# dashpay/agora-blsful

Measured on AMD Instinct MI355X. Metric: BLS12-381 sig verifications/sec (batch), higher is better.
Workload: dtype u32

## Files before the change

agora-blsful_amd/csrc/blsgpu.hip:

```cpp
#include <hip/hip_runtime.h>
#include <stdio.h>
#include <stdlib.h>
#include <string.h>
#include <algorithm>
#include <atomic>
#include <chrono>
#include <mutex>
#include <numeric>
#include <string>
#include <thread>
#include <type_traits>
#include <unordered_map>
#include <vector>

#include "../../include/blsgpu.h"
#include "kernels.cuh"
#include "shares.cuh"
#include "secure.cuh"
#include "agg_batch.cuh"
#include "host_sha256.h"

namespace {

const uint32_t FP_ONE_HOST[12] = FP_RAW_ONE_WORDS;
thread_local std::string t_err;
thread_local size_t t_devidx = 0;
thread_local bool t_nested = false;

enum {
  KID_PREPARE, KID_MILLER2, KID_FINALEXP, KID_PREPARE_AGG, KID_PAIRS_AFF, KID_MILLER1, KID_F12_FOLD, KID_FINALEXP_ONE,
  KID_HASH, KID_ACCUM, KID_POINT_FOLD, KID_COMPRESS, KID_SIGN, KID_F12_IO, KID_MSM_SORT, KID_MSM_BUCKET, KID_MSM_CHUNK, KID_DECOMPRESS, KID_PAIRING_COOP, KID_KEY_SORT, KID_COEFF, KID_DUP, KID_FIRST_BAD, KID_MSM_PREP, KID_MSM_NORM, KID_MSM_MERGE, KID_WIDE, KID_LINES, KID_CYCRUN,
  KID_MILLER2_V1, KID_FINALEXP_V1, KID_LINESP, KID_LINESP4, KID_LINE_QUAD, KID_F12_FOLD4, KID_F12_TREE, KID_HORNER, KID_MILLERFP, KID_PAIRING_POST, KID_PAIRING_PRE,
  KID_TAIL,
  KID_SHARE_LAGRANGE, KID_SHARE_LADDER, KID_SHARE_FOLD, KID_SHARE_OUT,
  KID_SECURE_RANK, KID_SECURE_GATHER, KID_SECURE_DIGEST, KID_SECURE_COEFF, KID_SECURE_OUT, KID_SECURE_FIN,
  KID_AGG_SEG_INDEX, KID_AGG_SEG_FOLD, KID_AGG_SEG_FIN,
  KID_COUNT
};
const char* KID_NAMES[KID_COUNT] = {"k_prepare", "k_millerf2s", "k_finalexp2s", "k_prepare_agg", "k_pairs_to_affine", "k_miller1s", "k_f12_fold",
                                    "k_finalexp_one", "k_hash_to_point", "k_accumulate", "k_point_fold", "k_compress", "k_sign", "k_f12_io", "k_msm_sort", "k_msm_bucket", "k_msm_chunk", "k_decompress", "k_pairing_coop", "k_key_sort", "k_sha256_coeff", "k_duplicate_rule", "k_first_identity", "k_msm_prep", "k_normalize", "k_msm_merge", "k_wide", "k_lines2s", "k_cyc_run4",
                                    "k_miller2s", "k_finalexps", "k_linesp", "k_linesp4", "k_line_quad", "k_f12_fold4", "k_f12_tree_seg", "k_f12_horner_wide", "k_millerfp", "k_pairing_post", "k_pairing_pre",
                                    "tail_stream_overlapped", "k_share_lagrange", "k_share_ladder", "k_share_fold", "k_share_out",
                                    "k_secure_rank", "k_secure_gather", "k_secure_digest", "k_secure_coeff", "k_secure_out", "k_secure_fin",
                                    "k_agg_seg_index", "k_f12_fold_seg", "k_agg_batch_fin"};

struct Ctx {
  int dev = -1;
  hipStream_t stream = nullptr;
  uint8_t* arena = nullptr;
  size_t arena_cap = 0, arena_off = 0;
  std::mutex mu;
  hipEvent_t ev_host = nullptr;
  hipStream_t side = nullptr;
  hipEvent_t ev_fork = nullptr, ev_join = nullptr;
  hipStream_t side2 = nullptr;
  hipEvent_t ev_join2 = nullptr;
  uint8_t* hpin = nullptr;
  size_t hpin_cap = 0;
  uint8_t* hsmall = nullptr;
  size_t hsmall_off = 0;
  hipStream_t tail = nullptr;
  hipEvent_t ev_tail_fork = nullptr, ev_tail_join = nullptr;
  uint32_t* fold_ws = nullptr;
  uint32_t* lines_ws = nullptr;
  size_t lines_cap = 0;
  uint32_t* stream_flags = nullptr;
  uint32_t stream_epoch = 0;
  bool prof_on = false;
  struct Pending { int kid; hipEvent_t e0, e1; };
  std::vector<Pending> prof_pending;
  std::vector<hipEvent_t> prof_pool;
  double prof_ms[KID_COUNT] = {0};
  uint64_t prof_cnt[KID_COUNT] = {0};
};
struct Device {
  int dev = -1;
  std::vector<Ctx*> pool;
// ... 34 lines not shown
  Ctx* c = d->pool[d->rr.fetch_add(1) % d->pool.size()];
  L.lk = std::unique_lock<std::mutex>(c->mu);
  L.c = c;
  return L;
}
#define CTX_ACQUIRE_ON(c, devidx)        \
  Lease lease_ = acquire_ctx(devidx);     \
  Ctx* c = lease_.c;                      \
  c->hsmall_off = 0;                      \
  HIPCK(hipSetDevice(c->dev))
#define CTX_ACQUIRE(c) CTX_ACQUIRE_ON(c, t_devidx)
#define NOT_INIT() fail(BLSGPU_E_NOT_INIT, "blsgpu_init has not been called (or found no gfx950 device)")
#define API_CATCH                                                                              \
  catch (const std::bad_alloc&) { return fail(BLSGPU_E_HIP, "out of host memory"); }           \
  catch (const std::exception& e) { return fail(BLSGPU_E_HIP, std::string("internal: ") + e.what()); } \
  catch (...) { return fail(BLSGPU_E_HIP, "internal: unknown exception"); }

int fail(int code, const std::string& msg) {
  t_err = msg;
  return code;
}
extern "C" char** environ;
struct Knobs {
  long coop_max = 4096, wide_max = 512, shard_min = 8192, contexts = 2, fake_devices = 0, acc_lanes = 57344;
  long msm_c = 0, msm_ch = 0, msm2_c = 0, msm2_ch = 0, msm2_q = 0;
  long msm2_tables = 1;
  long stream_lines = 1;
  long post_split = 3;
  long host_trace = 0, strict_env = 0, ab_knobs = 0;
  long shares_msm_min = 1024;
  long secure_batch_max = 1024;
  long agg_batch_max = 32768;
  long ws_keep_mb = 4096;
  long miller_chunk = 65536, miller_v1 = 0, row_pad = 192, wide_mode = 2, finalexp_seg = 0, finalexp_v1 = 0, prepare_lanes = 0, product_tree = 1,
       tree_local = 0, lines4_max = -1, tree_engine_from = 0, agg_lanes = 0, msm_v1 = 0, msm_naive = 0, wide_test_block = 64;
  std::string problem;
};
struct KnobSpec { const char* name; long Knobs::*field; long lo, hi; bool ab; };
const KnobSpec KNOB_TABLE[] = {
    {"BLSGPU_COOP_MAX", &Knobs::coop_max, 0, 1 << 20, false},          {"BLSGPU_WIDE_MAX", &Knobs::wide_max, 0, 4096, false},
    {"BLSGPU_SHARD_MIN", &Knobs::shard_min, 1, 1L << 40, false},        {"BLSGPU_CONTEXTS", &Knobs::contexts, 1, 16, false},
    {"BLSGPU_FAKE_DEVICES", &Knobs::fake_devices, 0, 64, false},        {"BLSGPU_ACC_LANES", &Knobs::acc_lanes, 64, 1 << 20, false},
    {"BLSGPU_MSM_C", &Knobs::msm_c, 4, 16, false},                      {"BLSGPU_MSM_CH", &Knobs::msm_ch, 1, 1 << 16, false},
    {"BLSGPU_MSM2_C", &Knobs::msm2_c, 4, 16, false},                    {"BLSGPU_MSM2_CH", &Knobs::msm2_ch, 1, 1 << 16, false},
    {"BLSGPU_MSM2_Q", &Knobs::msm2_q, 1, 8, false},                     {"BLSGPU_HOST_TRACE", &Knobs::host_trace, 0, 1, false},
    {"BLSGPU_WS_KEEP_MB", &Knobs::ws_keep_mb, 0, 1L << 20, false},        {"BLSGPU_MSM2_TABLES", &Knobs::msm2_tables, 0, 1, false},
    {"BLSGPU_STREAM_LINES", &Knobs::stream_lines, 0, 1, false},        {"BLSGPU_POST_SPLIT", &Knobs::post_split, 0, 3, false},
    {"BLSGPU_STRICT_ENV", &Knobs::strict_env, 0, 1, false},             {"BLSGPU_AB_KNOBS", &Knobs::ab_knobs, 0, 1, false},
    {"BLSGPU_SHARES_MSM_MIN", &Knobs::shares_msm_min, 2, 1L << 32, false},
    {"BLSGPU_SECURE_BATCH_MAX", &Knobs::secure_batch_max, 1, 1L << 32, false},
    {"BLSGPU_AGG_BATCH_MAX", &Knobs::agg_batch_max, 1, 1L << 32, false},
    {"BLSGPU_MILLER_CHUNK", &Knobs::miller_chunk, 0, 65536, true},      {"BLSGPU_MILLER_V1", &Knobs::miller_v1, 0, 1, true},
    {"BLSGPU_ROW_PAD", &Knobs::row_pad, 0, 4096, true},                 {"BLSGPU_WIDE_MODE", &Knobs::wide_mode, 1, 2, true},
    {"BLSGPU_FINALEXP_SEG", &Knobs::finalexp_seg, 0, 1, true},          {"BLSGPU_FINALEXP_V1", &Knobs::finalexp_v1, 0, 1, true},
    {"BLSGPU_PREPARE_LANES", &Knobs::prepare_lanes, 0, 2, true},        {"BLSGPU_PRODUCT_TREE", &Knobs::product_tree, 0, 1, true},
    {"BLSGPU_TREE_LOCAL", &Knobs::tree_local, 0, 65536, true},          {"BLSGPU_LINES4_MAX", &Knobs::lines4_max, 0, 65536, true},
    {"BLSGPU_TREE_ENGINE_FROM", &Knobs::tree_engine_from, 0, 256, true}, {"BLSGPU_AGG_LANES", &Knobs::agg_lanes, 0, 2, true},
    {"BLSGPU_MSM_V1", &Knobs::msm_v1, 0, 1, true},                      {"BLSGPU_MSM_NAIVE", &Knobs::msm_naive, 0, 1, true},
    {"BLSGPU_WIDE_TEST_BLOCK", &Knobs::wide_test_block, 64, 256, true},
};
const char* const KNOB_OTHER_NAMES[] = {"BLSGPU_LIB", "BLSGPU_HASH_STOP"};
Knobs parse_knobs() {
  Knobs k;
  const char* gate = getenv("BLSGPU_AB_KNOBS");
  const bool ab_ok = gate && atol(gate) == 1;
  for (const KnobSpec& sp : KNOB_TABLE) {
    const char* e = getenv(sp.name);
    if (!e || !*e) continue;
    if (sp.ab && !ab_ok) {
      if (k.problem.empty()) k.problem = std::string(sp.name) + " is an A/B switch and needs BLSGPU_AB_KNOBS=1";
      fprintf(stderr, "libblsgpu: ignoring %s (an A/B switch: set BLSGPU_AB_KNOBS=1 to honour it)\n", sp.name);
      continue;
    }
    char* end = nullptr;
    long v = strtol(e, &end, 10);
    if (end == e || *end) {
      if (k.problem.empty()) k.problem = std::string(sp.name) + " is not an integer";
      continue;
    }
    k.*sp.field = v < sp.lo ? sp.lo : v > sp.hi ? sp.hi : v;
  }
  for (char** e = environ; e && *e; e++) {
    if (strncmp(*e, "BLSGPU_", 7) != 0) continue;
    const char* eq = strchr(*e, '=');
    const std::string name(*e, eq ? (size_t)(eq - *e) : strlen(*e));
    bool known = false;
    for (const KnobSpec& sp : KNOB_TABLE) known = known || name == sp.name;
    for (const char* o : KNOB_OTHER_NAMES) known = known || name == o;
    if (!known && k.problem.empty()) k.problem = "unknown variable " + name;
  }
  return k;
}
// ... 385 lines not shown
    c->lines_cap = 0;
  }
}

void launch_finalexp_chunk(Ctx* c, size_t n, size_t first, size_t cnt, const uint32_t* d_f, int32_t* d_status, bool seg) {
  const size_t nlanes = lanes_for(cnt), lanes = row_stride(nlanes);
  const dim3 grid((unsigned)(nlanes / BLS_BLOCK));
  if (seg) {
    const dim3 grid4(blocks_for(4 * cnt));
    for (int s = 0; s <= 5; s++) {
      KL(KID_FINALEXP, k_finalexp_seg, grid, dim3(BLS_BLOCK), s, n, first, cnt, d_f, c->lines_ws, lanes, d_status);
      if (s < 5) KL(KID_CYCRUN, k_cyc_run4, grid4, dim3(BLS_BLOCK), cnt, c->lines_ws, lanes, (const int32_t*)d_status, first);
    }
  } else {
    KL(KID_FINALEXP, k_finalexp2s, grid, dim3(BLS_BLOCK), n, first, cnt, d_f, c->lines_ws, lanes, d_status);
  }
}

int run_pairing2(Ctx* c, size_t n, uint32_t* d_pairs, uint32_t* d_f, int32_t* d_status, int fixed_g2) {
  if (n <= wide_max_items() && n <= coop_max_items()) {
    if (knobs().wide_mode == 1) {
      uint32_t* d_easy = (uint32_t*)arena_take(c, (size_t)WIDE_EASY_WORDS * 4 * n);
      if (!d_easy) return fail(BLSGPU_E_HIP, "internal: arena too small");
      KL(KID_PAIRING_COOP, k_pairing_coop_easy, dim3((unsigned)n), dim3(BLS_BLOCK), n, (const uint32_t*)d_pairs, (const int32_t*)d_status, fixed_g2, d_easy);
      KL(KID_WIDE, k_finalexp_wide, dim3((unsigned)n), dim3(WIDE_ENGINE_BLOCK), n, (const uint32_t*)d_easy, d_status);
    } else {
      KL(KID_WIDE, k_pairing_wide, dim3((unsigned)n), dim3(WIDE_ENGINE_BLOCK), n, (const uint32_t*)d_pairs, d_status, fixed_g2);
    }
  } else if (n <= coop_max_items()) {
    KL(KID_PAIRING_COOP, k_pairing_coop, dim3((unsigned)n), dim3(BLS_BLOCK), n, d_pairs, d_status, fixed_g2);
  } else {
    const bool finalexp_seg = knobs().finalexp_seg != 0;
    const bool finalexp_v1 = knobs().finalexp_v1 != 0;
    const size_t chunk = n < miller_chunk_items() ? n : miller_chunk_items();
    const size_t words_per_lane = (size_t)MILLER_ENTRIES * (LINE5_WORDS + (fixed_g2 ? 0 : LINE3_WORDS_H));
    if (chunk && lines_reserve(c, words_per_lane * 4 * row_stride(lanes_for(chunk))) == 0) {
      for (size_t first = 0; first < n; first += chunk) {
        const size_t cnt = n - first < chunk ? n - first : chunk;
        const size_t nlanes = lanes_for(cnt), lanes = row_stride(nlanes);
        uint32_t* lines3 = c->lines_ws + (size_t)MILLER_ENTRIES * LINE5_WORDS * lanes;
        const dim3 grid((unsigned)(nlanes / BLS_BLOCK));
        if (fixed_g2) {
          KL(KID_LINES, k_lines2s, grid, dim3(BLS_BLOCK), n, first, cnt, (const uint32_t*)d_pairs, (const int32_t*)d_status, c->lines_ws, lines3, lanes, fixed_g2, 0);
        } else {
          KL(KID_LINES, k_lines2s, grid, dim3(BLS_BLOCK), n, first, cnt, (const uint32_t*)d_pairs, (const int32_t*)d_status, c->lines_ws, lines3, lanes, 0, 1);
          KL(KID_LINES, k_lines2s, grid, dim3(BLS_BLOCK), n, first, cnt, (const uint32_t*)d_pairs, (const int32_t*)d_status, c->lines_ws, lines3, lanes, 0, 2);
        }
        KL(KID_MILLER2, k_millerf2s, grid, dim3(BLS_BLOCK), n, first, cnt, (const int32_t*)d_status, (const uint32_t*)c->lines_ws, lanes, d_f);
        if (!finalexp_v1) launch_finalexp_chunk(c, n, first, cnt, d_f, d_status, finalexp_seg);
      }
      if (finalexp_v1) KL(KID_FINALEXP_V1, k_finalexps, dim3(blocks_for(2 * n)), dim3(BLS_BLOCK), n, d_f, d_status);
    } else {
      KL(KID_MILLER2_V1, k_miller2s, dim3(blocks_for(2 * n)), dim3(BLS_BLOCK), n, d_pairs, d_status, d_f, fixed_g2);
      KL(KID_FINALEXP_V1, k_finalexps, dim3(blocks_for(2 * n)), dim3(BLS_BLOCK), n, d_f, d_status);
    }
  }
  HIPCK(hipGetLastError());
  return 0;
}

int side_fork(Ctx* c, int which = 3) {
  if (!c->side) {
    HIPCK(hipStreamCreateWithFlags(&c->side, hipStreamNonBlocking));
    HIPCK(hipEventCreateWithFlags(&c->ev_fork, hipEventDisableTiming));
    HIPCK(hipEventCreateWithFlags(&c->ev_join, hipEventDisableTiming));
    HIPCK(hipStreamCreateWithFlags(&c->side2, hipStreamNonBlocking));
    HIPCK(hipEventCreateWithFlags(&c->ev_join2, hipEventDisableTiming));
  }
  if (which & 1) HIPCK(hipEventRecord(c->ev_fork, c->stream));
  if (which & 2) {
    HIPCK(hipStreamWaitEvent(c->side, c->ev_fork, 0));
    HIPCK(hipStreamWaitEvent(c->side2, c->ev_fork, 0));
  }
  return 0;
}

void launch_hash_g1_small(hipStream_t stream, size_t n, const uint8_t* d_msgs, const uint64_t* d_offs, int flags, const dst_arg& dst, uint8_t* d_out,
                          uint32_t* d_rec) {
  if (n <= 128 && hash_phase_stop() == 0)
// ... 981 lines not shown
      cnt += c->prof_cnt[kernel_id];
    }
  if (total_ms) *total_ms = ms;
  if (launches) *launches = cnt;
  return 0;
}
API_CATCH

size_t blsgpu_last_error(char* buf, size_t cap) {
  if (buf && cap) {
    size_t k = std::min(cap - 1, t_err.size());
    memcpy(buf, t_err.data(), k);
    buf[k] = 0;
  }
  return t_err.size();
}

int blsgpu_verify_batch(int sig_group, int scheme, const void* pks, const void* sigs, const uint8_t* msgs,
                        const uint64_t* msg_offsets, size_t n, int fmt, int32_t* status) try {
  const bool wire = fmt == BLSGPU_FMT_COMPRESSED || fmt == BLSGPU_FMT_LEGACY;
  int rc = check_common(sig_group, scheme, wire ? BLSGPU_FMT_RAW_PROJ : fmt);
  if (rc) return rc;
  if (n == 0) return 0;
  if (!pks || !sigs || !msg_offsets || !status) return fail(BLSGPU_E_ARG, "null argument");
  if (const size_t D = shard_devices(n, {pks, sigs, msgs, msg_offsets, status}); D > 1) {
    const size_t psz = pk_size(sig_group, fmt), ssz = sig_size(sig_group, fmt);
    return run_on_devices(D, [&](size_t d) {
      const size_t lo = n * d / D, hi = n * (d + 1) / D;
      return blsgpu_verify_batch(sig_group, scheme, (const uint8_t*)pks + lo * psz, (const uint8_t*)sigs + lo * ssz, msgs, msg_offsets + lo, hi - lo,
                                 fmt, status + lo);
    });
  }
  CTX_ACQUIRE(c);
  uint64_t total = 0;
  if (is_device_ptr(msg_offsets)) HIPCK(hipMemcpy(&total, msg_offsets + n, 8, hipMemcpyDeviceToHost));
  else total = msg_offsets[n];
  const size_t pkb = pk_size(sig_group, fmt) * n, sgb = sig_size(sig_group, fmt) * n;
  size_t need = pad256(pkb) + pad256(sgb) + pad256(total) + pad256(8 * (n + 1)) + pad256(4 * n) + 2 * pad256((size_t)WS_PAIRS_WORDS * 4 * n) + 4096 +
                (wire ? pad256(288 * n) + pad256(144 * n) : 0);
  rc = arena_reserve(c, need);
  if (rc) return rc;
  c->arena_off = 0;
  const void *d_pks, *d_sigs, *d_msgs, *d_offs;
  {
    const void* ptrs[4] = {pks, sigs, msgs, msg_offsets};
    const size_t sizes[4] = {pkb, sgb, (size_t)total, 8 * (n + 1)};
    const void* outs[4];
    if (stage_in_packed(c, ptrs, sizes, outs, 4)) {
      d_pks = outs[0];
      d_sigs = outs[1];
      d_msgs = outs[2];
      d_offs = outs[3];
    } else {
      if ((rc = stage_in(c, pks, pkb, &d_pks))) return rc;
      if ((rc = stage_in(c, sigs, sgb, &d_sigs))) return rc;
      if ((rc = stage_in(c, msgs, total, &d_msgs))) return rc;
      if ((rc = stage_in(c, msg_offsets, 8 * (n + 1), &d_offs))) return rc;
    }
  }
  int32_t* d_status = (int32_t*)arena_take(c, 4 * n);
  uint32_t* d_pairs = (uint32_t*)arena_take(c, (size_t)WS_PAIRS_WORDS * 4 * n);
  uint32_t* d_f = (uint32_t*)arena_take(c, (size_t)WS_F_WORDS * 4 * n);
  if (!d_status || !d_pairs || !d_f) return fail(BLSGPU_E_HIP, "internal: arena too small");
  int pre = 0, kfmt = fmt;
  if (wire) {
    uint8_t* d_pk_raw = (uint8_t*)arena_take(c, pk_size(sig_group, BLSGPU_FMT_RAW_PROJ) * n);
    uint8_t* d_sig_raw = (uint8_t*)arena_take(c, sig_size(sig_group, BLSGPU_FMT_RAW_PROJ) * n);
    if (!d_pk_raw || !d_sig_raw) return fail(BLSGPU_E_HIP, "internal: arena too small");
    const int legacy = fmt == BLSGPU_FMT_LEGACY;
    with_group(key_group(sig_group), [&](auto KG) {
      KL(KID_DECOMPRESS, k_decompress<KG()>, dim3(blocks_for(n)), dim3(BLS_BLOCK), n, (const uint8_t*)d_pks, legacy, d_pk_raw, d_status, 0);
      KL(KID_DECOMPRESS, k_decompress<3 - KG()>, dim3(blocks_for(n)), dim3(BLS_BLOCK), n, (const uint8_t*)d_sigs, legacy, d_sig_raw, d_status, 1);
    });
    d_pks = d_pk_raw;
    d_sigs = d_sig_raw;
    pre = 1;
    kfmt = BLSGPU_FMT_RAW_PROJ;
  }
  rc = run_verify_items(c, sig_group, scheme == BLSGPU_SCHEME_AUG, (const uint8_t*)d_pks, (const uint8_t*)d_sigs, kfmt,
                        (const uint8_t*)d_msgs, (const uint64_t*)d_offs, 0, scheme_dst(sig_group, scheme), n, d_pairs, d_f, d_status, pre);
  if (rc) return rc;
  if ((rc = status_out_and_sync(c, status, d_status, n))) return rc;
  return 0;
}
API_CATCH

int blsgpu_verify_batch_grouped(int sig_group, int scheme, const void* pks, const void* sigs, const uint8_t* msgs, const uint64_t* msg_offsets, size_t n,
                                int fmt, uint64_t seed, int32_t* status) try {
  int rc = check_common(sig_group, scheme, fmt);
// ... 1864 lines not shown
```

agora-blsful_amd/csrc/kernels.cuh:

```cuda
#pragma once
#ifndef BLS_SPLIT_WAVES
#define BLS_SPLIT_WAVES 2
#endif
#include "verify.cuh"

#define BLS_BLOCK 64
#define W1 FP_NL
#define W2 (2 * FP_NL)
#define WS_PAIRS_WORDS (6 * W2)
#define WS_PAIR1_WORDS (3 * W2)
#define WS_F_WORDS (6 * W2)
#define LINE5_WORDS (5 * FP_NL)
#define LINE3_WORDS_H (3 * FP_NL)
#define FX_STORE_WORDS (10 * 6 * FP_NL)
#define MILLER1_GROUP 3

struct dst_arg {
  uint8_t b[256];
  uint32_t len;
};

__device__ __forceinline__ void ws_ld_fp(fp& r, const uint32_t* ws, size_t stride, size_t i, int w0) {
#pragma unroll
  for (int k = 0; k < FP_NL; k++) r.l[k] = (int32_t)ws[(size_t)(w0 + k) * stride + i];
}
__device__ __forceinline__ void ws_st_fp(uint32_t* ws, size_t stride, size_t i, int w0, const fp& a) {
#pragma unroll
  for (int k = 0; k < FP_NL; k++) ws[(size_t)(w0 + k) * stride + i] = (uint32_t)a.l[k];
}
__device__ __forceinline__ void ws_ld_fp2(fp2& r, const uint32_t* ws, size_t stride, size_t i, int w0) {
  ws_ld_fp(r.c0, ws, stride, i, w0);
  ws_ld_fp(r.c1, ws, stride, i, w0 + W1);
}
__device__ __forceinline__ void ws_st_fp2(uint32_t* ws, size_t stride, size_t i, int w0, const fp2& a) {
  ws_st_fp(ws, stride, i, w0, a.c0);
  ws_st_fp(ws, stride, i, w0 + W1, a.c1);
}
// ... 159 lines not shown
    }
  }
}


__device__ __forceinline__ void scalar_load_mod_r(uint32_t v[8], const uint8_t* scalars, size_t i) {
  const uint32_t* k = (const uint32_t*)(scalars + 32 * i);
#pragma unroll
  for (int j = 0; j < 8; j++) v[j] = k[j];
  const uint32_t R[8] = {0x00000001u, 0xffffffffu, 0xfffe5bfeu, 0x53bda402u, 0x09a1d805u, 0x3339d808u, 0x299d7d48u, 0x73eda753u};
  for (int round = 0; round < 3; round++) {
    uint32_t d[8];
    uint64_t bw = 0;
#pragma unroll
    for (int j = 0; j < 8; j++) {
      const uint64_t t = (uint64_t)v[j] - R[j] - bw;
      d[j] = (uint32_t)t;
      bw = (t >> 63) & 1;
    }
    if (!bw) {
#pragma unroll
      for (int j = 0; j < 8; j++) v[j] = d[j];
    }
  }
}

template <int SG>
__global__ void k_prepare(size_t n, const uint8_t* pks, const uint8_t* sigs, int fmt, int aug, const uint8_t* msgs,
                          const uint64_t* offs, int single_msg, dst_arg dst, uint32_t* pairs, int32_t* status, int pre_status, int two_lanes);
__global__ void k_miller2s(size_t n, const uint32_t* pairs, const int32_t* status, uint32_t* fws, int fixed_g2);
__global__ void k_lines2s(size_t n, size_t first, size_t count, const uint32_t* pairs, const int32_t* status, uint32_t* lines, uint32_t* lines3, size_t lanes, int fixed_g2, int pass);
__global__ void k_millerf2s(size_t n, size_t first, size_t count, const int32_t* status, const uint32_t* lines, size_t lanes, uint32_t* fws);
__global__ void k_finalexp2s(size_t n, size_t first, size_t count, const uint32_t* fws, uint32_t* vp, size_t lanes, int32_t* status);
__global__ void k_finalexp_seg(int seg, size_t n, size_t first, size_t count, const uint32_t* fws, uint32_t* vp, size_t lanes, int32_t* status);
__global__ void k_cyc_run4(size_t count, uint32_t* vp, size_t lanes, const int32_t* status, size_t first);
__global__ void k_linesp(size_t mm, size_t half, size_t stride, const uint32_t* pairs, const int32_t* bad, uint32_t* lines, uint32_t* lines3, size_t lanes, size_t first_v, size_t count_v, int pass);
__global__ void k_linesp4(size_t cnt, size_t stride, const uint32_t* pairs, const int32_t* bad, uint32_t* lines3, size_t lanes);
__global__ void k_lines_fixed(size_t stride, const uint32_t* pairs, const int32_t* bad, uint32_t* lines3, size_t lanes, int fixed_g2);
__global__ void k_millerfp(size_t count_v, size_t q, int group, const uint32_t* lines, size_t lanes, uint32_t* fws, size_t stride, size_t out0);
__global__ void k_millerfp3(size_t count, size_t q, int group, const int32_t* bad, const uint32_t* lines3, size_t lanes, uint32_t* fws, size_t stride, size_t out0);
__global__ void k_line_quad(size_t count, size_t q, const int32_t* bad, const uint32_t* lines3, size_t lanes, uint32_t* fout, size_t sout, size_t rout, size_t oout);
__global__ void k_f12_fold4(size_t qin, size_t qout, int fan, const uint32_t* fin, size_t sin, size_t rin, uint32_t* fout, size_t sout, size_t rout, size_t oout);
__global__ void k_finalexps(size_t n, const uint32_t* fws, int32_t* status);
__global__ void k_miller1s(size_t n, size_t stride, const uint32_t* pairs, const int32_t* skip, uint32_t* fws);
__global__ void k_finalexp_ones(const uint32_t* fws, size_t stride, int32_t* verdict);
__global__ void k_pairing_coop(size_t n, const uint32_t* pairs, int32_t* status, int fixed_g2);
__global__ void k_finalexp_coop(const uint32_t* fws, size_t stride, int32_t* verdict);
template <int SG>
__global__ void k_prepare_agg(size_t n, const uint8_t* pks, const uint8_t* sig, int fmt, int aug, const uint8_t* msgs,
                              const uint64_t* offs, dst_arg dst, uint32_t* pairs, int32_t* bad, int two_lanes, int has_sig);
__global__ void k_pairs_to_affine(size_t n, const uint8_t* g1s, const uint8_t* g2s, int fmt, uint32_t* pairs, int32_t* skip);
__global__ void k_pairs2_to_affine(size_t n, const uint8_t* g1a, const uint8_t* g2a, const uint8_t* g1b, const uint8_t* g2b, int fmt,
                                   uint32_t* pairs, int32_t* status);
__global__ void k_status_to_flag(size_t n, int32_t* status);
template <int SG>
__global__ void k_prepare_hashed(size_t n, const uint8_t* pks, const uint8_t* sigs, const uint8_t* hashes, uint32_t* pairs, int32_t* status, int fmt);
template <int SG>
__global__ void k_prepare_proof(size_t n, const uint8_t* commitments, const uint8_t* proofs, const uint8_t* pks, const uint8_t* ys,
                                int fmt, const uint8_t* msgs, const uint64_t* offs, dst_arg dst, uint32_t* pairs, int32_t* status);
__global__ void k_f12_fold(size_t m, size_t half, uint32_t* fws, size_t stride);
#define GROUPED_ITEMS 8
template <int SG>
__global__ void k_prepare_grouped(size_t n, const uint8_t* pks, const uint8_t* sigs, int fmt, int aug, const uint8_t* msgs, const uint64_t* offs,
                                  dst_arg dst, uint64_t seed, size_t ng, uint32_t* pairs, int32_t* skip, uint8_t* scaled_sigs, int32_t* status);
__global__ void k_group_sigsum(size_t ng, size_t n, const uint8_t* scaled_sigs, uint32_t* pairs, int32_t* skip);
__global__ void k_f12_mul3(size_t ng, const uint32_t* fin, size_t stride_in, uint32_t* fout);
// ... 1291 lines not shown
  {
    hfp2 q;
    fp p;
    ws_ld_hfp2(q, pairs, stride, j, W2);
    ls_st(sh, L4_X, q.v);
    ws_ld_hfp2(q, pairs, stride, j, 2 * W2);
    ls_st(sh, L4_Y, q.v);
    fp2_one(q);
    ls_st(sh, L4_Z, q.v);
    ws_ld_fp(p, pairs, stride, j, 0);
    ls_st(sh, L4_PX, p);
    ws_ld_fp(p, pairs, stride, j, W1);
    ls_st(sh, L4_PY, p);
  }
  for (int e = 0; e < MILLER_ENTRIES; e++) {
    if (miller_entry_is_add(e)) lines4_add_fn(sh, pairs, stride, j, lines3, lanes, t2, e, pr);
    else lines4_dbl_fn(sh, lines3, lanes, t2, e, pr);
  }
}
#endif

#if defined(BLS_TU_MILLERF)
static __device__ __noinline__ void f12_sh_sqr_fn(lds_u32* sh) {
  fp12_t<hfp2> a, r;
  sh_ld_f12(a, sh);
  fp12_sqr_body(r, a);
  sh_st_f12(sh, r);
}
static __device__ __noinline__ void f12_sh_mul_line5_fn(lds_u32* sh, const uint32_t* lines, size_t lanes, uint32_t t, int e) {
  line5_t<hfp2> L;
  line5_ld(L, lines, lanes, t, e);
  f12_sh_mul_line5(sh, L);
}
__global__ void __launch_bounds__(BLS_BLOCK, BLS_SPLIT_WAVES) __attribute__((disable_tail_calls))
k_millerf2s(size_t n, size_t first, size_t count, const int32_t* status, const uint32_t* lines, size_t lanes, uint32_t* fws) {
  const uint32_t t = blockIdx.x * BLS_BLOCK + threadIdx.x;
  const size_t j = t >> 1;
  if (j >= count) return;
  const size_t i = first + j;
  if (status[i] != BLS_OK) return;
  __shared__ uint32_t fsh[F12_SH_WORDS * BLS_BLOCK];
  f12_sh acc = {lds_column(fsh)};
  line5_t<hfp2> L;
  line5_ld(L, lines, lanes, t, 0);
  acc_set_line5(acc, L);
  for (int e = 1; e < MILLER_ENTRIES; e++) {
    if (!miller_entry_is_add(e)) f12_sh_sqr_fn(acc.sh);
    f12_sh_mul_line5_fn(acc.sh, lines, lanes, t, e);
  }
  fp12_t<hfp2> f;
  sh_ld_f12(f, acc.sh);
  fp12_conj(f, f);
  ws_st_hfp12(fws, n, i, f);
}
#endif

#if defined(BLS_TU_FINALEXPS)
__global__ void __launch_bounds__(BLS_BLOCK, BLS_SPLIT_WAVES) k_finalexp_ones(const uint32_t* fws, size_t stride, int32_t* verdict) {
  if (blockIdx.x != 0 || threadIdx.x >= 2) return;
  fp12_t<hfp2> f;
  ws_ld_hfp12(f, fws, stride, 0);
  int st = pairing_verdict(f);
  if (!lane_hi()) *verdict = st;
}
__global__ void __launch_bounds__(BLS_BLOCK, BLS_SPLIT_WAVES) k_finalexps(size_t n, const uint32_t* fws, int32_t* status) {
  size_t i = ((size_t)blockIdx.x * blockDim.x + threadIdx.x) >> 1;
  if (i >= n) return;
  if (status[i] != BLS_OK) return;
  fp12_t<hfp2> f;
  ws_ld_hfp12(f, fws, n, i);
  int st = pairing_verdict(f);
  if (!lane_hi()) status[i] = st;
}
#endif

#if defined(BLS_TU_MILLERF)
__global__ void __launch_bounds__(BLS_BLOCK, BLS_SPLIT_WAVES) __attribute__((disable_tail_calls))
k_millerfp(size_t count_v, size_t q, int group, const uint32_t* lines, size_t lanes, uint32_t* fws, size_t stride, size_t out0) {
  const uint32_t t = blockIdx.x * BLS_BLOCK + threadIdx.x;
  const size_t g = t >> 1;
  if (g >= q) return;
  const uint32_t hi = t & 1u;
  __shared__ uint32_t fsh[F12_SH_WORDS * BLS_BLOCK];
  f12_sh acc = {lds_column(fsh)};
  {
    line5_t<hfp2> L;
    line5_ld(L, lines, lanes, (uint32_t)(2 * g) + hi, 0);
    acc_set_line5(acc, L);
  }
  for (int e = 0; e < MILLER_ENTRIES; e++) {
    if (e > 0 && !miller_entry_is_add(e)) f12_sh_sqr_fn(acc.sh);
    for (int k = e == 0 ? 1 : 0; k < group; k++) {
      const size_t v = g + (size_t)k * q;
      if (v < count_v) f12_sh_mul_line5_fn(acc.sh, lines, lanes, (uint32_t)(2 * v) + hi, e);
    }
  }
  fp12_t<hfp2> f;
  sh_ld_f12(f, acc.sh);
  fp12_conj(f, f);
  ws_st_hfp12(fws, stride, out0 + g, f);
}
#endif

#if defined(BLS_TU_MILLERF)
static __device__ __noinline__ void f12_sh_mul_line3_fn(lds_u32* sh, const uint32_t* lines3, size_t lanes, uint32_t t, int e) {
  hfp2 l0, l2, l3;
  fp* c[3] = {&l0.v, &l2.v, &l3.v};
  lanes = uni_sz(lanes);
  gc_u32* row = uni_global(lines3) + (size_t)uni_u32((uint32_t)e) * (3 * FP_NL) * lanes;
#pragma unroll
  for (int j = 0; j < 3; j++)
#pragma unroll
    for (int k = 0; k < FP_NL; k++) {
      c[j]->l[k] = (int32_t)g_ld_nt(row, t);
      row += lanes;
    }
  f12_sh_mul_line3(sh, l0, l2, l3);
}
__global__ void __launch_bounds__(BLS_BLOCK, BLS_SPLIT_WAVES) __attribute__((disable_tail_calls))
k_millerfp3(size_t count, size_t q, int group, const int32_t* bad, const uint32_t* lines3, size_t lanes, uint32_t* fws, size_t stride, size_t out0) {
  const uint32_t t = blockIdx.x * BLS_BLOCK + threadIdx.x;
  const size_t g = t >> 1;
  if (g >= q) return;
  const uint32_t hi = t & 1u;
  __shared__ uint32_t fsh[F12_SH_WORDS * BLS_BLOCK];
  f12_sh acc = {lds_column(fsh)};
  acc_one(acc);
  for (int e = 0; e < MILLER_ENTRIES; e++) {
    if (e > 0 && !miller_entry_is_add(e)) f12_sh_sqr_fn(acc.sh);
    for (int k = 0; k < group; k++) {
      const size_t v = g + (size_t)k * q;
      if (v < count && bad[v] == 0) f12_sh_mul_line3_fn(acc.sh, lines3, lanes, (uint32_t)(2 * v) + hi, e);
    }
  }
  fp12_t<hfp2> f;
  sh_ld_f12(f, acc.sh);
  fp12_conj(f, f);
  ws_st_hfp12(fws, stride, out0 + g, f);
}
#endif

#if defined(BLS_TU_MILLERF)
static __device__ __noinline__ void f12_sh_st_ws_fn(lds_u32* sh, uint32_t* ws, size_t stride, uint32_t off);
__device__ __forceinline__ void quad_line_ld(hfp2& l0, hfp2& l2, hfp2& l3, size_t count, const int32_t* bad, gc_u32* row, size_t lanes, size_t x, uint32_t hi) {
  if (x < count && bad[x] == 0) {
    fp* c[3] = {&l0.v, &l2.v, &l3.v};
    const uint32_t t = (uint32_t)(2 * x) + hi;
#pragma unroll
    for (int j = 0; j < 3; j++)
#pragma unroll
      for (int k = 0; k < FP_NL; k++) {
        c[j]->l[k] = (int32_t)g_ld_nt(row, t);
        row += lanes;
      }
  } else {
    fp2_one(l0);
    fp2_zero(l2);
    fp2_zero(l3);
  }
}
template <int FIRST>
static __device__ __noinline__ void quad_merge_fn(lds_u32* sh, size_t count, const int32_t* bad, const uint32_t* row_, size_t lanes, size_t xa, size_t xb, uint32_t hi) {
  hfp2 a0, a2, a3, b0, b2, b3;
  gc_u32* row = uni_global(row_);
  lanes = uni_sz(lanes);
  quad_line_ld(a0, a2, a3, count, bad, row, lanes, xa, hi);
  quad_line_ld(b0, b2, b3, count, bad, row, lanes, xb, hi);
  line5_t<hfp2> L;
  lines_merge(L, a0, a2, a3, b0, b2, b3);
  if (FIRST) {
    f12_sh acc = {sh};
    acc_set_line5(acc, L);
  } else {
    f12_sh_mul_line5(sh, L);
  }
// ... 360 lines not shown
#if BLS_CYC_KARA
  if (fx_pow_finish_n<4, 0>(sh, vp, lanes, t)) {
    fx_store(sh, vp, lanes, t, 6);
    for (int j = 0; j < 3; j++) fx_cyc_sqr(sh);
    fx_mul(sh, vp, lanes, t, 6, FX_CONJ);
    fx_pow_finish_n<4, 1>(sh, vp, lanes, t);
  } else {
    fx_pow_plain(sh, vp, lanes, t);
  }
#else
  if (!fx_pow_finish(sh, vp, lanes, t)) fx_pow_plain(sh, vp, lanes, t);
#endif
  fx_conj(sh);
}
static __device__ __noinline__ int fx_is_one(lds_u32* sh) {
  fp12_t<hfp2> a;
  sh_ld_f12(a, sh);
  return fp12_is_one(a) ? BLS_OK : BLS_ERR_INVALID_SIGNATURE;
}
static __device__ __noinline__ int fx_eq_conj(lds_u32* sh, uint32_t* vp, size_t lanes, uint32_t t, int slot) {
  const vs_ref v = {vp, lanes, t};
  bool eq = true, zero = true;
#pragma unroll
  for (int j = 0; j < 6; j++) {
    hfp2 a, b;
    sh_ld_fp(a.v, sh, 13 * j);
    vs_ld(b.v, v, slot, j);
    if (j >= 3) fp2_neg(b, b);
    eq = fp2_eq(a, b) && eq;
    zero = fp2_is_zero(b) && zero;
  }
  return eq && !zero ? BLS_OK : BLS_ERR_INVALID_SIGNATURE;
}
__global__ void __launch_bounds__(BLS_BLOCK, BLS_SPLIT_WAVES) __attribute__((disable_tail_calls))
k_finalexp2s(size_t n, size_t first, size_t count, const uint32_t* fws, uint32_t* vp, size_t lanes, int32_t* status) {
  const uint32_t t = blockIdx.x * BLS_BLOCK + threadIdx.x;
  const size_t j = t >> 1;
  if (j >= count) return;
  const size_t i = first + j;
  if (status[i] != BLS_OK) return;
  __shared__ uint32_t ash[F12_SH_WORDS * BLS_BLOCK];
  lds_u32* sh = lds_column(ash);
  {
    fp12_t<hfp2> f;
    ws_ld_hfp12(f, fws, n, i);
    fp12_reduce(f, f);
    sh_st_f12(sh, f);
  }
  fx_store(sh, vp, lanes, t, 1);
  fx_inv(sh);
  fx_store(sh, vp, lanes, t, 0);
  fx_load(sh, vp, lanes, t, 1, FX_CONJ);
  fx_mul(sh, vp, lanes, t, 0, FX_PLAIN);
  fx_store(sh, vp, lanes, t, 1);
  fx_frob2(sh);
  fx_mul(sh, vp, lanes, t, 1, FX_PLAIN);
  fx_store(sh, vp, lanes, t, 1);
  fx_pow_x(sh, vp, lanes, t);
  fx_mul(sh, vp, lanes, t, 1, FX_CONJ);
  fx_store(sh, vp, lanes, t, 0);
  fx_pow_x(sh, vp, lanes, t);
  fx_mul(sh, vp, lanes, t, 0, FX_CONJ);
  fx_store(sh, vp, lanes, t, 0);
  fx_pow_x(sh, vp, lanes, t);
  fx_mul(sh, vp, lanes, t, 0, FX_FROB1);
  fx_store(sh, vp, lanes, t, 0);
  fx_pow_x(sh, vp, lanes, t);
  fx_pow_x(sh, vp, lanes, t);
  fx_mul(sh, vp, lanes, t, 0, FX_FROB2);
  fx_mul(sh, vp, lanes, t, 0, FX_CONJ);
  fx_store(sh, vp, lanes, t, 0);
  fx_load(sh, vp, lanes, t, 1, FX_PLAIN);
  fx_cyc_sqr(sh);
  fx_mul(sh, vp, lanes, t, 0, FX_PLAIN);
  const int st = fx_eq_conj(sh, vp, lanes, t, 1);
  if (!lane_hi()) status[i] = st;
}
__device__ __forceinline__ void fx_pow_end(lds_u32* sh, uint32_t* vp, size_t lanes, uint32_t t) {
  if (!fx_pow_finish(sh, vp, lanes, t)) fx_pow_plain(sh, vp, lanes, t);
  fx_conj(sh);
}
__global__ void __launch_bounds__(BLS_BLOCK, BLS_SPLIT_WAVES) __attribute__((disable_tail_calls))
k_finalexp_seg(int seg, size_t n, size_t first, size_t count, const uint32_t* fws, uint32_t* vp, size_t lanes, int32_t* status) {
  const uint32_t t = blockIdx.x * BLS_BLOCK + threadIdx.x;
  const size_t j = t >> 1;
  if (j >= count) return;
  const size_t i = first + j;
  if (status[i] != BLS_OK) return;
  __shared__ uint32_t ash[F12_SH_WORDS * BLS_BLOCK];
  lds_u32* sh = lds_column(ash);
  if (seg == 0) {
    {
      fp12_t<hfp2> f;
      ws_ld_hfp12(f, fws, n, i);
      fp12_reduce(f, f);
      sh_st_f12(sh, f);
    }
    fx_store(sh, vp, lanes, t, 1);
    fx_inv(sh);
    fx_store(sh, vp, lanes, t, 0);
    fx_load(sh, vp, lanes, t, 1, FX_CONJ);
    fx_mul(sh, vp, lanes, t, 0, FX_PLAIN);
    fx_store(sh, vp, lanes, t, 1);
    fx_frob2(sh);
    fx_mul(sh, vp, lanes, t, 1, FX_PLAIN);
    fx_store(sh, vp, lanes, t, 1);
    fx_store(sh, vp, lanes, t, 2);
    return;
  }
  fx_pow_end(sh, vp, lanes, t);
  if (seg == 1 || seg == 2) {
    fx_mul(sh, vp, lanes, t, seg == 1 ? 1 : 0, FX_CONJ);
  } else if (seg == 3) {
    fx_mul(sh, vp, lanes, t, 0, FX_FROB1);
  } else if (seg == 5) {
    fx_mul(sh, vp, lanes, t, 0, FX_FROB2);
    fx_mul(sh, vp, lanes, t, 0, FX_CONJ);
    fx_store(sh, vp, lanes, t, 0);
    fx_load(sh, vp, lanes, t, 1, FX_PLAIN);
    fx_cyc_sqr(sh);
    fx_mul(sh, vp, lanes, t, 1, FX_PLAIN);
    fx_mul(sh, vp, lanes, t, 0, FX_PLAIN);
    const int st = fx_is_one(sh);
    if (!lane_hi()) status[i] = st;
    return;
  }
  if (seg != 4) fx_store(sh, vp, lanes, t, 0);
  fx_store(sh, vp, lanes, t, 2);
}
#endif

#if defined(BLS_TU_CYCRUN4)
#if !defined(BLS_TU_FINALEXP2)
#define VS_WORDS (6 * FP_NL)
__device__ __forceinline__ void cpow_slot(int k, int j, int& slot, int& idx) {
  const int q = 4 * k + j;
  slot = 3 + q / 6;
  idx = q % 6;
}
#endif
__device__ __forceinline__ int32_t dpp_cross(int32_t x) { return __builtin_amdgcn_mov_dpp(x, 0x4E, 0xF, 0xF, true); }
__device__ __forceinline__ void fp_cross(fp& r, const fp& a) {
#pragma unroll
  for (int i = 0; i < FP_NL; i++) r.l[i] = dpp_cross(a.l[i]);
}
__device__ __forceinline__ void cyc_store_signed(lds_u32* sh, int w0, const hfp2& u, const hfp2& z, bool plus) {
  hfp2 zz, nz, r;
  fp2_neg(nz, z);
  fp_sel(zz.v, plus, z.v, nz.v);
  fp2_add(r, u, zz);
  fp2_dbl(r, r);
  fp2_add(r, r, u);
  fp2_reduce(r, r);
  sh_st_fp(sh, w0, r.v);
}
static __device__ __noinline__ void cyc4_sqr_fn(lds_u32* sh, bool pair_b) {
  hfp2 a, b, t0, t1, r0, r1, x, u0, u1;
  sh_ld_fp(a.v, sh, 0);
  sh_ld_fp(b.v, sh, 13);
  fp4_sqr(t0, t1, a, b);
  fp_cross(r0.v, t0.v);
  fp_cross(r1.v, t1.v);
// ... 1633 lines not shown
```

Baseline: 3.454 million.

## Fuse Miller loop and final exponentiation into one verify kernel

Adds a k_millerfx2s kernel, built in a new translation unit, that runs the Miller loop from the precomputed lines and then the final exponentiation verdict in the same kernel. The Fp12 value stays in LDS instead of being written to and reread from the fws workspace, and one kernel launch per chunk goes away. It becomes the default path unless TAIL_V1, finalexp_seg or finalexp_v1 is set. Separately, the verify entry now skips staging and reading the offset total when msgs is already a device pointer. The fused kernel may use more registers or lower occupancy, which could offset the saved traffic.

```diff
diff --git a/agora-blsful_amd/csrc/blsgpu.hip b/agora-blsful_amd/csrc/blsgpu.hip
--- a/agora-blsful_amd/csrc/blsgpu.hip
+++ b/agora-blsful_amd/csrc/blsgpu.hip
@@ -35,6 +35,7 @@
   KID_SHARE_LAGRANGE, KID_SHARE_LADDER, KID_SHARE_FOLD, KID_SHARE_OUT,
   KID_SECURE_RANK, KID_SECURE_GATHER, KID_SECURE_DIGEST, KID_SECURE_COEFF, KID_SECURE_OUT, KID_SECURE_FIN,
   KID_AGG_SEG_INDEX, KID_AGG_SEG_FOLD, KID_AGG_SEG_FIN,
+  KID_MILLERFX,
   KID_COUNT
 };
 const char* KID_NAMES[KID_COUNT] = {"k_prepare", "k_millerf2s", "k_finalexp2s", "k_prepare_agg", "k_pairs_to_affine", "k_miller1s", "k_f12_fold",
@@ -42,7 +43,7 @@
                                     "k_miller2s", "k_finalexps", "k_linesp", "k_linesp4", "k_line_quad", "k_f12_fold4", "k_f12_tree_seg", "k_f12_horner_wide", "k_millerfp", "k_pairing_post", "k_pairing_pre",
                                     "tail_stream_overlapped", "k_share_lagrange", "k_share_ladder", "k_share_fold", "k_share_out",
                                     "k_secure_rank", "k_secure_gather", "k_secure_digest", "k_secure_coeff", "k_secure_out", "k_secure_fin",
-                                    "k_agg_seg_index", "k_f12_fold_seg", "k_agg_batch_fin"};
+                                    "k_agg_seg_index", "k_f12_fold_seg", "k_agg_batch_fin", "k_millerfx2s"};
 
 struct Ctx {
   int dev = -1;
@@ -143,7 +144,7 @@
   long secure_batch_max = 1024;
   long agg_batch_max = 32768;
   long ws_keep_mb = 4096;
-  long miller_chunk = 65536, miller_v1 = 0, row_pad = 192, wide_mode = 2, finalexp_seg = 0, finalexp_v1 = 0, prepare_lanes = 0, product_tree = 1,
+  long miller_chunk = 65536, miller_v1 = 0, row_pad = 192, wide_mode = 2, finalexp_seg = 0, finalexp_v1 = 0, tail_v1 = 0, prepare_lanes = 0, product_tree = 1,
        tree_local = 0, lines4_max = -1, tree_engine_from = 0, agg_lanes = 0, msm_v1 = 0, msm_naive = 0, wide_test_block = 64;
   std::string problem;
 };
@@ -168,7 +169,7 @@
     {"BLSGPU_TREE_LOCAL", &Knobs::tree_local, 0, 65536, true},          {"BLSGPU_LINES4_MAX", &Knobs::lines4_max, 0, 65536, true},
     {"BLSGPU_TREE_ENGINE_FROM", &Knobs::tree_engine_from, 0, 256, true}, {"BLSGPU_AGG_LANES", &Knobs::agg_lanes, 0, 2, true},
     {"BLSGPU_MSM_V1", &Knobs::msm_v1, 0, 1, true},                      {"BLSGPU_MSM_NAIVE", &Knobs::msm_naive, 0, 1, true},
-    {"BLSGPU_WIDE_TEST_BLOCK", &Knobs::wide_test_block, 64, 256, true},
+    {"BLSGPU_WIDE_TEST_BLOCK", &Knobs::wide_test_block, 64, 256, true}, {"BLSGPU_TAIL_V1", &Knobs::tail_v1, 0, 1, true},
 };
 const char* const KNOB_OTHER_NAMES[] = {"BLSGPU_LIB", "BLSGPU_HASH_STOP"};
 Knobs parse_knobs() {
@@ -620,6 +621,7 @@
   } else {
     const bool finalexp_seg = knobs().finalexp_seg != 0;
     const bool finalexp_v1 = knobs().finalexp_v1 != 0;
+    const bool fused_tail = !knobs().tail_v1 && !finalexp_seg && !finalexp_v1;
     const size_t chunk = n < miller_chunk_items() ? n : miller_chunk_items();
     const size_t words_per_lane = (size_t)MILLER_ENTRIES * (LINE5_WORDS + (fixed_g2 ? 0 : LINE3_WORDS_H));
     if (chunk && lines_reserve(c, words_per_lane * 4 * row_stride(lanes_for(chunk))) == 0) {
@@ -633,6 +635,10 @@
         } else {
           KL(KID_LINES, k_lines2s, grid, dim3(BLS_BLOCK), n, first, cnt, (const uint32_t*)d_pairs, (const int32_t*)d_status, c->lines_ws, lines3, lanes, 0, 1);
           KL(KID_LINES, k_lines2s, grid, dim3(BLS_BLOCK), n, first, cnt, (const uint32_t*)d_pairs, (const int32_t*)d_status, c->lines_ws, lines3, lanes, 0, 2);
+        }
+        if (fused_tail) {
+          KL(KID_MILLERFX, k_millerfx2s, grid, dim3(BLS_BLOCK), first, cnt, (const uint32_t*)c->lines_ws, c->lines_ws, lanes, d_status);
+          continue;
         }
         KL(KID_MILLER2, k_millerf2s, grid, dim3(BLS_BLOCK), n, first, cnt, (const int32_t*)d_status, (const uint32_t*)c->lines_ws, lanes, d_f);
         if (!finalexp_v1) launch_finalexp_chunk(c, n, first, cnt, d_f, d_status, finalexp_seg);
@@ -1680,9 +1686,12 @@
     });
   }
   CTX_ACQUIRE(c);
+  const bool dev_msgs = is_device_ptr(msgs);
   uint64_t total = 0;
-  if (is_device_ptr(msg_offsets)) HIPCK(hipMemcpy(&total, msg_offsets + n, 8, hipMemcpyDeviceToHost));
-  else total = msg_offsets[n];
+  if (!dev_msgs) {
+    if (is_device_ptr(msg_offsets)) HIPCK(hipMemcpy(&total, msg_offsets + n, 8, hipMemcpyDeviceToHost));
+    else total = msg_offsets[n];
+  }
   const size_t pkb = pk_size(sig_group, fmt) * n, sgb = sig_size(sig_group, fmt) * n;
   size_t need = pad256(pkb) + pad256(sgb) + pad256(total) + pad256(8 * (n + 1)) + pad256(4 * n) + 2 * pad256((size_t)WS_PAIRS_WORDS * 4 * n) + 4096 +
                 (wire ? pad256(288 * n) + pad256(144 * n) : 0);
@@ -1694,7 +1703,7 @@
     const void* ptrs[4] = {pks, sigs, msgs, msg_offsets};
     const size_t sizes[4] = {pkb, sgb, (size_t)total, 8 * (n + 1)};
     const void* outs[4];
-    if (stage_in_packed(c, ptrs, sizes, outs, 4)) {
+    if (!dev_msgs && stage_in_packed(c, ptrs, sizes, outs, 4)) {
       d_pks = outs[0];
       d_sigs = outs[1];
       d_msgs = outs[2];
@@ -1702,7 +1711,8 @@
     } else {
       if ((rc = stage_in(c, pks, pkb, &d_pks))) return rc;
       if ((rc = stage_in(c, sigs, sgb, &d_sigs))) return rc;
-      if ((rc = stage_in(c, msgs, total, &d_msgs))) return rc;
+      if (dev_msgs) d_msgs = msgs;
+      else if ((rc = stage_in(c, msgs, total, &d_msgs))) return rc;
       if ((rc = stage_in(c, msg_offsets, 8 * (n + 1), &d_offs))) return rc;
     }
   }
diff --git a/agora-blsful_amd/csrc/kernels.cuh b/agora-blsful_amd/csrc/kernels.cuh
--- a/agora-blsful_amd/csrc/kernels.cuh
+++ b/agora-blsful_amd/csrc/kernels.cuh
@@ -3,6 +3,10 @@
 #define BLS_SPLIT_WAVES 2
 #endif
 #include "verify.cuh"
+#if defined(BLS_TU_MILLERFX)
+#define BLS_TU_MILLERF 1
+#define BLS_TU_FINALEXP2 1
+#endif
 
 #define BLS_BLOCK 64
 #define W1 FP_NL
@@ -228,6 +232,7 @@
 __global__ void k_lines2s(size_t n, size_t first, size_t count, const uint32_t* pairs, const int32_t* status, uint32_t* lines, uint32_t* lines3, size_t lanes, int fixed_g2, int pass);
 __global__ void k_millerf2s(size_t n, size_t first, size_t count, const int32_t* status, const uint32_t* lines, size_t lanes, uint32_t* fws);
 __global__ void k_finalexp2s(size_t n, size_t first, size_t count, const uint32_t* fws, uint32_t* vp, size_t lanes, int32_t* status);
+__global__ void k_millerfx2s(size_t first, size_t count, const uint32_t* lines, uint32_t* vp, size_t lanes, int32_t* status);
 __global__ void k_finalexp_seg(int seg, size_t n, size_t first, size_t count, const uint32_t* fws, uint32_t* vp, size_t lanes, int32_t* status);
 __global__ void k_cyc_run4(size_t count, uint32_t* vp, size_t lanes, const int32_t* status, size_t first);
 __global__ void k_linesp(size_t mm, size_t half, size_t stride, const uint32_t* pairs, const int32_t* bad, uint32_t* lines, uint32_t* lines3, size_t lanes, size_t first_v, size_t count_v, int pass);
@@ -1585,6 +1590,7 @@
   line5_ld(L, lines, lanes, t, e);
   f12_sh_mul_line5(sh, L);
 }
+#if !defined(BLS_TU_MILLERFX)
 __global__ void __launch_bounds__(BLS_BLOCK, BLS_SPLIT_WAVES) __attribute__((disable_tail_calls))
 k_millerf2s(size_t n, size_t first, size_t count, const int32_t* status, const uint32_t* lines, size_t lanes, uint32_t* fws) {
   const uint32_t t = blockIdx.x * BLS_BLOCK + threadIdx.x;
@@ -1607,6 +1613,7 @@
   ws_st_hfp12(fws, n, i, f);
 }
 #endif
+#endif
 
 #if defined(BLS_TU_FINALEXPS)
 __global__ void __launch_bounds__(BLS_BLOCK, BLS_SPLIT_WAVES) k_finalexp_ones(const uint32_t* fws, size_t stride, int32_t* verdict) {
@@ -1627,7 +1634,7 @@
 }
 #endif
 
-#if defined(BLS_TU_MILLERF)
+#if defined(BLS_TU_MILLERF) && !defined(BLS_TU_MILLERFX)
 __global__ void __launch_bounds__(BLS_BLOCK, BLS_SPLIT_WAVES) __attribute__((disable_tail_calls))
 k_millerfp(size_t count_v, size_t q, int group, const uint32_t* lines, size_t lanes, uint32_t* fws, size_t stride, size_t out0) {
   const uint32_t t = blockIdx.x * BLS_BLOCK + threadIdx.x;
@@ -1655,7 +1662,7 @@
 }
 #endif
 
-#if defined(BLS_TU_MILLERF)
+#if defined(BLS_TU_MILLERF) && !defined(BLS_TU_MILLERFX)
 static __device__ __noinline__ void f12_sh_mul_line3_fn(lds_u32* sh, const uint32_t* lines3, size_t lanes, uint32_t t, int e) {
   hfp2 l0, l2, l3;
   fp* c[3] = {&l0.v, &l2.v, &l3.v};
@@ -1693,7 +1700,7 @@
 }
 #endif
 
-#if defined(BLS_TU_MILLERF)
+#if defined(BLS_TU_MILLERF) && !defined(BLS_TU_MILLERFX)
 static __device__ __noinline__ void f12_sh_st_ws_fn(lds_u32* sh, uint32_t* ws, size_t stride, uint32_t off);
 __device__ __forceinline__ void quad_line_ld(hfp2& l0, hfp2& l2, hfp2& l3, size_t count, const int32_t* bad, gc_u32* row, size_t lanes, size_t x, uint32_t hi) {
   if (x < count && bad[x] == 0) {
@@ -2120,21 +2127,7 @@
   }
   return eq && !zero ? BLS_OK : BLS_ERR_INVALID_SIGNATURE;
 }
-__global__ void __launch_bounds__(BLS_BLOCK, BLS_SPLIT_WAVES) __attribute__((disable_tail_calls))
-k_finalexp2s(size_t n, size_t first, size_t count, const uint32_t* fws, uint32_t* vp, size_t lanes, int32_t* status) {
-  const uint32_t t = blockIdx.x * BLS_BLOCK + threadIdx.x;
-  const size_t j = t >> 1;
-  if (j >= count) return;
-  const size_t i = first + j;
-  if (status[i] != BLS_OK) return;
-  __shared__ uint32_t ash[F12_SH_WORDS * BLS_BLOCK];
-  lds_u32* sh = lds_column(ash);
-  {
-    fp12_t<hfp2> f;
-    ws_ld_hfp12(f, fws, n, i);
-    fp12_reduce(f, f);
-    sh_st_f12(sh, f);
-  }
+__device__ __forceinline__ int fx_verdict(lds_u32* sh, uint32_t* vp, size_t lanes, uint32_t t) {
   fx_store(sh, vp, lanes, t, 1);
   fx_inv(sh);
   fx_store(sh, vp, lanes, t, 0);
@@ -2161,7 +2154,25 @@
   fx_load(sh, vp, lanes, t, 1, FX_PLAIN);
   fx_cyc_sqr(sh);
   fx_mul(sh, vp, lanes, t, 0, FX_PLAIN);
-  const int st = fx_eq_conj(sh, vp, lanes, t, 1);
+  return fx_eq_conj(sh, vp, lanes, t, 1);
+}
+#if !defined(BLS_TU_MILLERFX)
+__global__ void __launch_bounds__(BLS_BLOCK, BLS_SPLIT_WAVES) __attribute__((disable_tail_calls))
+k_finalexp2s(size_t n, size_t first, size_t count, const uint32_t* fws, uint32_t* vp, size_t lanes, int32_t* status) {
+  const uint32_t t = blockIdx.x * BLS_BLOCK + threadIdx.x;
+  const size_t j = t >> 1;
+  if (j >= count) return;
+  const size_t i = first + j;
+  if (status[i] != BLS_OK) return;
+  __shared__ uint32_t ash[F12_SH_WORDS * BLS_BLOCK];
+  lds_u32* sh = lds_column(ash);
+  {
+    fp12_t<hfp2> f;
+    ws_ld_hfp12(f, fws, n, i);
+    fp12_reduce(f, f);
+    sh_st_f12(sh, f);
+  }
+  const int st = fx_verdict(sh, vp, lanes, t);
   if (!lane_hi()) status[i] = st;
 }
 __device__ __forceinline__ void fx_pow_end(lds_u32* sh, uint32_t* vp, size_t lanes, uint32_t t) {
@@ -2216,6 +2227,35 @@
   if (seg != 4) fx_store(sh, vp, lanes, t, 0);
   fx_store(sh, vp, lanes, t, 2);
 }
+#else
+static __device__ __noinline__ void fx_seam(lds_u32* sh) {
+  fp12_t<hfp2> f;
+  sh_ld_f12(f, sh);
+  fp12_conj(f, f);
+  fp12_reduce(f, f);
+  sh_st_f12(sh, f);
+}
+__global__ void __launch_bounds__(BLS_BLOCK, BLS_SPLIT_WAVES) __attribute__((disable_tail_calls))
+k_millerfx2s(size_t first, size_t count, const uint32_t* lines, uint32_t* vp, size_t lanes, int32_t* status) {
+  const uint32_t t = blockIdx.x * BLS_BLOCK + threadIdx.x;
+  const size_t j = t >> 1;
+  if (j >= count) return;
+  const size_t i = first + j;
+  if (status[i] != BLS_OK) return;
+  __shared__ uint32_t fsh[F12_SH_WORDS * BLS_BLOCK];
+  f12_sh acc = {lds_column(fsh)};
+  line5_t<hfp2> L;
+  line5_ld(L, lines, lanes, t, 0);
+  acc_set_line5(acc, L);
+  for (int e = 1; e < MILLER_ENTRIES; e++) {
+    if (!miller_entry_is_add(e)) f12_sh_sqr_fn(acc.sh);
+    f12_sh_mul_line5_fn(acc.sh, lines, lanes, t, e);
+  }
+  fx_seam(acc.sh);
+  const int st = fx_verdict(acc.sh, vp, lanes, t);
+  if (!lane_hi()) status[i] = st;
+}
+#endif
 #endif
 
 #if defined(BLS_TU_CYCRUN4)
diff --git a/agora-blsful_amd/csrc/tu_millerfx.hip b/agora-blsful_amd/csrc/tu_millerfx.hip
--- /dev/null
+++ b/agora-blsful_amd/csrc/tu_millerfx.hip
@@ -0,0 +1,2 @@
+#define BLS_TU_MILLERFX 1
+#include "kernels.cuh"
```

New measurement: 3.428 million. No clear change (-0.7%).
